# zhengxwen/HIBAG

Measured on AMD Instinct MI355X. Metric: hlaPredict() samples/sec, 10k samples x 100-classifier HLA-B, higher is better.
Workload: dtype f64; 1 GPU; BASELINE config 2: synthetic hla-b model (50 alleles, 100 classifiers, 150 SNPs, 505000 haplotype-pair evaluations/sample), 10000 samples per GPU per step, type=response+dosage, vote=prob; genotypes and outputs resident in HBM (transfers excluded: `host_inclusive` is the PCIe-inclusive rate of the host-pointer entry); samples_per_gpu=10000, parallelism=sample-sharded x1 (contiguous slices, no collective), kernel_target=HIP, gfx950:sramecc+:xnack-, AMD Radeon Graphics, 256 CUs, engine=mfma (FP4 / int8 MFMA distances + FP64 VALU accumulation in reference order)

## Files before the change

### hibag_amd/_lib.py

```python

from __future__ import annotations

import ctypes as C
import os
import subprocess

_HERE = os.path.dirname(os.path.abspath(__file__))
CSRC = os.path.join(_HERE, "csrc")
LIB_PATH = os.environ.get("HIBAG_HIP_LIBRARY") or os.path.join(CSRC, "libhibag_hip.so")

K_PACK, K_TOTAL, K_ACCUM, K_FINISH, K_COUNT = 0, 1, 2, 3, 4
KERNEL_NAMES = {K_PACK: "pack", K_TOTAL: "total", K_ACCUM: "accum", K_FINISH: "finish"}

EXPORTS = [
    "hibag_hip_abi_version", "hibag_hip_last_error", "hibag_hip_device_count", "hibag_hip_set_device", "hibag_hip_get_device",
    "hibag_hip_set_kernel_target", "hibag_hip_model_new", "hibag_hip_model_add_classifier",
    "hibag_hip_model_add_classifier_packed", "hibag_hip_model_finalize", "hibag_hip_model_free",
    "hibag_hip_model_n_hla", "hibag_hip_model_n_snp", "hibag_hip_model_n_classifier",
    "hibag_hip_model_pair_evals", "hibag_hip_model_stored_cells", "hibag_hip_model_second_pass_pairs", "hibag_hip_model_mutation_table", "hibag_hip_predict",
    "hibag_hip_predict_device", "hibag_hip_model_set_snp_weights", "hibag_hip_predict_partial_device",
    "hibag_hip_finish_device", "hibag_hip_set_timing", "hibag_hip_get_timing", "hibag_hip_reset_timing",
    "hibag_hip_gpu_ext_proc", "hibag_hip_bed_flag", "hibag_hip_conv_bed", "hibag_hip_predict_bed", "hibag_hip_predict_mapped", "hibag_hip_predict_mapped_device",
    "hibag_hip_predict_snp_major", "hibag_hip_predict_snp_major_device",
    "hibag_hip_trainer_new", "hibag_hip_trainer_free", "hibag_hip_trainer_set_rng", "hibag_hip_trainer_set_seed",
    "hibag_hip_trainer_new_classifiers", "hibag_hip_trainer_n_classifier", "hibag_hip_trainer_classifier_dims",
    "hibag_hip_trainer_classifier_get", "hibag_hip_trainer_set_threads", "hibag_hip_trainer_threads", "hibag_hip_trainer_set_em_mode",
    "hibag_hip_trainer_set_shared", "hibag_hip_train_set_thread_budget", "hibag_hip_train_combine_stats", "hibag_hip_train_combine_times",
    "hibag_hip_model_status", "hibag_hip_model_clear_status", "hibag_hip_model_handover_faults",
    "hibag_hip_test_inject_handover_fault", "hibag_hip_model_engine", "hibag_hip_model_replicate",
    "hibag_hip_multi_slice", "hibag_hip_predict_multi", "hibag_hip_model_device",
    "hibag_hip_shard_bounds", "hibag_hip_model_shard", "hibag_hip_model_batch_limit", "hibag_hip_shard_group_new",
    "hibag_hip_shard_group_free", "hibag_hip_shard_group_ranks", "hibag_hip_shard_group_allreduces", "hibag_hip_rccl_version",
    "hibag_hip_shard_group_predict", "hibag_hip_predict_multi_sharded", "hibag_hip_measure_issue_costs",
    "hibag_hip_test_time_avg_prob", "hibag_hip_test_read_diag", "hibag_hip_plugin_degraded_calls", "hibag_hip_predict_oob",
    "hibag_hip_ld_geno_new", "hibag_hip_ld_geno_free", "hibag_hip_ld_snp_counts", "hibag_hip_ld_matrix", "hibag_hip_ld_gram_ms",
    "hibag_hip_ld_hla", "hibag_hip_model_distance", "hibag_hip_model_distance_ms",
    "hibag_hip_merge_plan_new", "hibag_hip_merge_plan_free", "hibag_hip_merge_device", "hibag_hip_predict_merge",
    "hibag_hip_predict_merge_bed", "hibag_hip_predict_prefix", "hibag_hip_predict_prefix_ms",
    "hibag_hip_predict_topk", "hibag_hip_predict_topk_device", "hibag_hip_predict_topk_mapped",
    "hibag_hip_predict_topk_snp_major", "hibag_hip_predict_topk_bed",
    "hibag_hip_cohort_new", "hibag_hip_cohort_from_bed", "hibag_hip_cohort_free", "hibag_hip_cohort_device",
    "hibag_hip_cohort_n_samp", "hibag_hip_cohort_n_snp", "hibag_hip_cohort_bytes", "hibag_hip_cohort_snp_counts",
    "hibag_hip_predict_cohort", "hibag_hip_predict_topk_cohort", "hibag_hip_predict_masked",
    "hibag_hip_test_build_eval_batch",
]
TOPK_MAX = 16


class HibagHipError(RuntimeError):
    def __init__(self, code: int, message: str):
        super().__init__(message or f"libhibag_hip error {code}")
        self.code = code


def build(force: bool = False) -> str:
    cmd = ["make", "-C", CSRC, "-s", "-j2"] + (["-B"] if force else [])
    subprocess.check_call(cmd)
    return LIB_PATH


_lib = None


def lib() -> C.CDLL:
    global _lib
    if _lib is not None:
        return _lib
# ... 110 lines not shown
    L.hibag_hip_model_engine.argtypes = [vp, i32, C.POINTER(i32), C.POINTER(i32)]
    L.hibag_hip_model_replicate.argtypes = [vp, i32]
    L.hibag_hip_model_replicate.restype = vp
    L.hibag_hip_multi_slice.argtypes = [i32, i32, i32, C.POINTER(i32), C.POINTER(i32)]
    L.hibag_hip_predict_multi.argtypes = [C.POINTER(vp), i32, vp, i32, i32, vp, vp, vp, vp, vp, vp]
    L.hibag_hip_shard_bounds.argtypes = [i32, i32, i32, C.POINTER(i32), C.POINTER(i32)]
    L.hibag_hip_model_shard.argtypes = [vp, i32, i32, i32]
    L.hibag_hip_model_shard.restype = vp
    L.hibag_hip_model_batch_limit.argtypes = [vp]
    L.hibag_hip_shard_group_new.argtypes = [C.POINTER(vp), i32]
    L.hibag_hip_shard_group_new.restype = vp
    L.hibag_hip_shard_group_free.argtypes = [vp]
    L.hibag_hip_shard_group_free.restype = None
    L.hibag_hip_shard_group_ranks.argtypes = [vp]
    L.hibag_hip_shard_group_allreduces.argtypes = [vp]
    L.hibag_hip_shard_group_allreduces.restype = i64
    L.hibag_hip_rccl_version.restype = i32
    L.hibag_hip_shard_group_predict.argtypes = [vp, vp, i32, vp, vp, vp, vp, vp, vp]
    L.hibag_hip_predict_multi_sharded.argtypes = [C.POINTER(vp), i32, vp, i32, vp, vp, vp, vp, vp, vp]
    L.hibag_hip_measure_issue_costs.argtypes = [C.POINTER(dbl)] * 4
    L.hibag_hip_test_time_avg_prob.argtypes = [vp, vp, i32, i32, i32, vp, vp, C.POINTER(dbl)]
    if hasattr(L, "hibag_hip_test_build_eval_batch"):
        L.hibag_hip_test_build_eval_batch.argtypes = [i32, i32, vp, vp, i32, i32, vp, vp, vp, vp, i32, vp, i32, vp, vp]
    if hasattr(L, "hibag_hip_test_read_diag"):
        L.hibag_hip_test_read_diag.argtypes = [vp, vp, i32]
        L.hibag_hip_plugin_degraded_calls.restype = i64
    _lib = L
    return L


def check(rc: int) -> None:
    if rc != 0:
        raise HibagHipError(rc, lib().hibag_hip_last_error().decode("utf-8", "replace"))
```

### hibag_amd/csrc/hibag_internal.h

```cpp
#ifndef HIBAG_INTERNAL_H_
#define HIBAG_INTERNAL_H_

#include <hip/hip_runtime.h>
#include <algorithm>
#include <chrono>
#include <cmath>
#include <cstdarg>
#include <cstdio>
#include <cstdlib>
#include <cstring>
#include <mutex>
#include <new>
#include <string>
#include <thread>
#include <vector>

#include "../../include/hibag_hip.h"
#include "hibag_device.h"
#include "hibag_kernels.h"
#include "hibag_plugin.h"

int hibag_fail(int code, const char *fmt, ...);
int hibag_selected_device();

// ... 122 lines not shown

}
using namespace hibag_detail;

struct hibag_hip_model {
	int device = 0;
	int n_hla = 0, n_snp = 0;
	bool finalized = false;
	bool have_snpidx = true;
	bool use_mfma = true;
	bool use_fp4 = true;
	std::vector<HostClassifier> cls;
	std::vector<int> snp_weight_override;
	int64_t pair_evals = 0;
	double tab[HIBAG_TAB_N];

	DevBuf d_int, d_stream, d_tile, d_tab, d_blk, d_pfac, d_phdr, d_parow;
	HibagModelView view{};
	int mask_rows = 0, bt_rows = 0, cell_rows = 0;
	size_t stream_bytes = 0;

	DevBuf ws_planes, ws_cw, ws_tot, ws_inv, ws_winv, ws_part, ws_best, ws_vrec, ws_geno, ws_out, ws_codes, ws_bt, ws_bias, ws_cells, ws_sync;
	std::vector<int> engine_of, steps_of;
	int store_mode = 0;
	int64_t second_pass_pairs = 0;
	HibagSideStream side;
	uint32_t epoch = 0;
	int *h_err = nullptr;
	DevBuf ws_err;
	int fault = 0;
	int64_t fault_count = 0;
	bool no_chunks = false;
	int drop_next = 0;
	uint32_t spin_limit = 1u << 19;
	hipEvent_t ws_done = nullptr;
	bool ws_pending = false;
	StagedStreams staged;
	PinBuf pin_geno, pin_out;
	bool staged_ready = false;
	DevBuf ws_bed, ws_bedidx;
	DevBuf oob_hap;
	size_t oob_freq_at = 0, oob_off_at = 0, oob_start_at = 0;
	bool oob_hap_ready = false;
	hipStream_t dist_st = nullptr;
	hipEvent_t dist_ev[2] = {nullptr, nullptr};
	DevBuf dist_cells, dist_tri, dist_acc, dist_num, dist_out;
// ... 84 lines not shown
```

### hibag_amd/csrc/hibag_k_pass1.h

```cpp
#ifndef HIBAG_K_PASS1_H_
#define HIBAG_K_PASS1_H_

__device__ __forceinline__ double *cell_rows(const HibagModelView &M, const HibagBatchView &B, int c, int group)
{
	return B.cells + ((size_t)group * (size_t)M.cell_row[M.n_classifier] + (size_t)M.cell_row[c]) * HIBAG_WAVE;
}

template <int NWP>
__device__ __forceinline__ double classifier_total(const HibagModelView &M, const HibagBatchView &B,
	int c, int s, int i0, int i1, int chunk0, double *__restrict__ rows, const double *tab_s)
{
	LaneMask<NWP> L;
	load_masks<NWP>(B, M.mask_row[c], s, L);
	const uint32_t *__restrict__ cnt = M.cls_cnt + M.cls_off[c];
	const uint32_t *__restrict__ cp = M.stream + M.stream_off[c] + (size_t)chunk0 * HIBAG_CHUNK_DWORDS(NWP);
	double total = 0;
	uint32_t n = cnt[i0];
	for (int i = i0; i < i1; i++) {
		const uint32_t n_next = cnt[i + 1];
		const double cell = cell_sum<NWP>(n, cp, L, tab_s);
		if (rows) __builtin_nontemporal_store(cell, &rows[(size_t)i * HIBAG_WAVE + (s & 63)]);
		total += cell;
		n = n_next;
	}
// ... 177 lines not shown
	double cell = 0, total = 0;
	double *__restrict__ rows = cell_rows(M, B, c, group);
	int row = seg[1];
	auto fin = [&](double v, bool, int) {
		__builtin_nontemporal_store(v, &rows[(size_t)row * HIBAG_WAVE + lane]); row++;
		if (WHOLE) { total += v; asm("" : "+v"(total)); }
	};
	const WideSrc wide = wide_src(B, M.bt_row[c], M.n_step[c], group);
	LaneOperand T;
	load_operand_row<HIBAG_ENGINE_FP4W>(B, M.bt_row[c], c, group, lane, T);
	ListCursor cur;
	walk_blocks<HIBAG_ENGINE_FP4W, TOTAL_G, false>(M, M.wide_seg_off[blockIdx.y], seg[2], lane, cur, hap_rsrc(M, M.hap_off[c]),
		M.n_snp_c[c] - HIBAG_FP4_STEP_SNPS * (wide.nstep - 1), T, wide, tab_s, cell, fin);
	if (WHOLE) {
		const size_t at = (size_t)c * B.n_pad + s;
		const double inv = 1 / total;
		B.tot[at] = total;
		B.inv[at] = inv;
		B.winv[2 * at + 1] = B.cw[at] > 0 ? inv : 0.0;
		note_infinite_reciprocal(B, c, s, B.cw[at], inv);
	}
}

__global__ void k_total_scan(HibagModelView M, HibagBatchView B)
{
	const int c = M.split_cls[blockIdx.y];
	const int s = blockIdx.x * blockDim.x + threadIdx.x;
	if (s >= B.n_pad) return;
	const double *__restrict__ rows = cell_rows(M, B, c, s >> 6) + (s & 63);
	const int n = M.cls_n[c];
	double total = 0;
	int i = 0;
	for (; i + 32 <= n; i += 32) {
		double v[32];
#pragma unroll
		for (int j = 0; j < 32; j++) v[j] = rows[(size_t)(i + j) * HIBAG_WAVE];
#pragma unroll
		for (int j = 0; j < 32; j++) total += v[j];
	}
	for (; i < n; i++) total += rows[(size_t)i * HIBAG_WAVE];
	B.tot[(size_t)c * B.n_pad + s] = total;
	B.inv[(size_t)c * B.n_pad + s] = 1 / total;
	B.winv[2 * ((size_t)c * B.n_pad + s) + 1] = B.cw[(size_t)c * B.n_pad + s] > 0 ? 1 / total : 0.0;
	note_infinite_reciprocal(B, c, s, B.cw[(size_t)c * B.n_pad + s], 1 / total);
}

template <int NB = 16>
__device__ __forceinline__ void ensemble_scalars(const HibagModelView &M, const HibagBatchView &B, int s, const int *__restrict__ best_cell)
{
	double sum_w = 0, sum_m = 0, num_m = 0;
	for (int c0 = 0; c0 < M.n_classifier; c0 += NB) {
		double wv[NB], tv[NB];
		int bv[NB];
#pragma unroll
		for (int j = 0; j < NB; j++) {
			const bool in = c0 + j < M.n_classifier;
			const size_t at = (size_t)(in ? c0 + j : c0) * B.n_pad + s;
			wv[j] = in ? B.cw[at] : 0.0;
			tv[j] = B.tot[at];
			bv[j] = best_cell ? best_cell[at] : 0;
		}
#pragma unroll
		for (int j = 0; j < NB; j++) {
// ... 23 lines not shown
```

### hibag_amd/csrc/hibag_kernels.hip

```cpp

#include <hip/hip_runtime.h>
#include <stdint.h>
#include <stdlib.h>
#include <string.h>
#include <algorithm>
#include "hibag_device.h"
#include "hibag_kernels.h"

#define NA_INTEGER (-2147483647 - 1)
#define CH HIBAG_CHUNK
#define BLOCK_WAVES HIBAG_BLOCK_WAVES
#define BLOCK_THREADS (BLOCK_WAVES * HIBAG_WAVE)
#ifndef TOTAL_G
#define TOTAL_G 8
#endif
#ifndef HIBAG_TOT_OCC
#define HIBAG_TOT_OCC 5
#endif
#ifndef HIBAG_TOT_OCC_MANY
#define HIBAG_TOT_OCC_MANY 6
#endif
#ifndef ACCUM_AHEAD
#define ACCUM_AHEAD true
#endif
// ... 94 lines not shown
{
	total[0] = resident_blocks(k_total<false, HIBAG_TOT_OCC, 0>, BLOCK_THREADS);
	total[1] = resident_blocks(k_total<false, HIBAG_TOT_OCC_MANY, 2>, BLOCK_THREADS);
	total[2] = resident_blocks(k_total<true, HIBAG_TOT_OCC, 0>, BLOCK_THREADS);
	total[3] = resident_blocks(k_total<true, HIBAG_TOT_OCC_MANY, 2>, BLOCK_THREADS);
	*accum = resident_blocks(k_accum, ACCUM_WAVES * HIBAG_WAVE);
}

void hibag_launch_total(const HibagModelView &M, const HibagBatchView &B, hipStream_t st, const HibagSideStream &side, bool vote)
{
	if (M.n_classifier == 0) return;
	const bool wide = M.n_wide > 0;
	if (wide) {
		const unsigned gq = (unsigned)((B.n_pad / HIBAG_WAVE + BLOCK_WAVES - 1) / BLOCK_WAVES);
		HibagModelView W = M;
		W.split_cls = M.wide_scan;
		const hipStream_t ws = side.stream ? side.stream : st;
		if (side.stream) {
			(void)hipEventRecord(side.fork, st);
			(void)hipStreamWaitEvent(side.stream, side.fork, 0);
		}
		if (M.n_wide_seg > 0 && M.n_wide_scan < M.n_wide) hipLaunchKernelGGL(k_total_wide<true>, dim3(gq, M.n_wide_seg), dim3(BLOCK_THREADS), 0, ws, M, B);
		else if (M.n_wide_seg > 0) hipLaunchKernelGGL(k_total_wide<false>, dim3(gq, M.n_wide_seg), dim3(BLOCK_THREADS), 0, ws, M, B);
		if (M.n_wide_scan > 0) hipLaunchKernelGGL(k_total_scan, dim3(B.n_pad / 64, M.n_wide_scan), dim3(64), 0, ws, W, B);
		if (side.stream) (void)hipEventRecord(side.join, side.stream);
	}
	if (M.n_item_whole == 0) {
		if (wide && side.stream) (void)hipStreamWaitEvent(st, side.join, 0);
		return;
	}
	const unsigned gx = (unsigned)((B.n_pad / HIBAG_WAVE + BLOCK_WAVES - 1) / BLOCK_WAVES);
	HibagModelView V = M;
	const double groups = (double)(B.n_pad / HIBAG_WAVE);
	const bool split = M.n_split > 0 && 1.25 * M.split_heavy_ns > M.split_rest_ns * groups / 4096.0;
	V.item = split ? M.item_split : M.item_whole;
	V.n_item = split ? M.n_item_split : M.n_item_whole;
	if (!split) V.n_split = 0;
	const unsigned n = gx * (unsigned)V.n_item;
	const int sbase = (M.store_cells && !vote) ? 2 : 0;
	const int slots_many = M.slots_total[sbase + 1];
	const bool many = M.all_fp4 && !split && slots_many > 0 && n >= 2u * (unsigned)slots_many;
	const int slots = M.slots_total[sbase + (many ? 1 : 0)];
	unsigned n_whole = n, rest = 0, stride = 8, K = 1;
	const int k_pass1 = tail_chunks(B.tail_k, M.p1_blocks / std::max(M.n_classifier, 1));
	if (!vote && k_pass1 > 1 && slots > 0 && n > (unsigned)slots) {
		K = (unsigned)k_pass1;
		rest = n % (unsigned)slots + (unsigned)slots;
		n_whole = n - rest;
		stride = (rest + 7) / 8 * 8;
	}
	const dim3 grid(n_whole + (rest ? K * stride : 0));
#define LAUNCH_TOTAL(STORE, OCC, WALK, VOTE) hipLaunchKernelGGL((k_total<STORE, OCC, WALK, VOTE>), grid, dim3(BLOCK_THREADS), 0, st, V, B, (int)gx, (int)n_whole, (int)rest, (int)stride, (int)K)
#define LAUNCH_WALK(STORE, VOTE) do { if (!many) LAUNCH_TOTAL(STORE, HIBAG_TOT_OCC, 0, VOTE);                                 \
		else if (M.p1_prebuilt) LAUNCH_TOTAL(STORE, HIBAG_TOT_OCC_MANY, 2, VOTE); else LAUNCH_TOTAL(STORE, HIBAG_TOT_OCC_MANY, 1, VOTE); } while (0)
	if (vote) LAUNCH_WALK(false, true);
	else if (M.store_cells) LAUNCH_WALK(true, false);
	else LAUNCH_WALK(false, false);
#undef LAUNCH_WALK
#undef LAUNCH_TOTAL
	if (split)
		hipLaunchKernelGGL(k_total_scan, dim3(B.n_pad / 64, V.n_split), dim3(64), 0, st, V, B);
	if (wide && side.stream) (void)hipStreamWaitEvent(st, side.join, 0);
}

void hibag_launch_accum(const HibagModelView &M, const HibagBatchView &B, hipStream_t st)
{
	if (M.store_cells == 1 && M.n_classifier > 0) {
		const unsigned groups_x = (unsigned)((B.n_pad / HIBAG_WAVE + 7) / 8), tq = (unsigned)((M.n_tile + CELLS_WAVES - 1) / CELLS_WAVES);
		hipLaunchKernelGGL(k_accum_cells, dim3(8 * groups_x * tq), dim3(CELLS_WAVES * HIBAG_WAVE), 0, st, M, B);
		return;
	}
	const unsigned n_group = (unsigned)(B.n_pad / HIBAG_WAVE);
	const unsigned n = 8u * (((n_group + 7) / 8 + ACCUM_WAVES - 1) / ACCUM_WAVES) * (unsigned)M.n_tile;
	if (n == 0 || M.n_classifier == 0) {
		(void)hipMemsetAsync(B.part, 0, (size_t)M.n_cell * B.n_pad * sizeof(double), st);
		return;
	}
	const int slots = M.slots_accum;
	const unsigned nx = n / 8, sx = (unsigned)slots / 8;
	unsigned n_whole = nx, K = 1;
	if (tail_chunks(B.tail_k, 0, 2) > 1 && sx > 0 && nx > sx) {
		K = (unsigned)tail_chunks(B.tail_k, 0, 2);
		n_whole = nx - (nx % sx + sx);
	}
// ... 77 lines not shown
```

### hibag_amd/csrc/hibag_model.hip

```cpp

#include "hibag_internal.h"

namespace hibag_detail {

void build_table(double *tab)
{
	const double min_rare_freq = 1e-5;
	for (int i = 0; i < HIBAG_TAB_N; i++) tab[i] = std::exp(i * std::log(min_rare_freq));
	tab[0] = 1;
	for (int i = 0; i < HIBAG_TAB_N; i++)
		if (!std::isfinite(tab[i])) tab[i] = 0;
}

int check_classifier_args(hibag_hip_model *m, int n_snp_c, const int32_t *snpidx, int n_haplo,
	const double *freq, const int32_t *hla)
{
	if (!m) return hibag_fail(HIBAG_HIP_EINVAL, "model is NULL");
	if (m->finalized) return hibag_fail(HIBAG_HIP_ESTATE, "model already finalized");
	if (n_snp_c < 0 || n_snp_c > HIBAG_HIP_MAX_SNP_IN_CLASSIFIER)
		return hibag_fail(HIBAG_HIP_EINVAL, "there are too many SNP markers in a classifier (%d > %d).",
			n_snp_c, HIBAG_HIP_MAX_SNP_IN_CLASSIFIER);
	if (n_haplo < 0 || (n_haplo > 0 && (!freq || !hla)))
		return hibag_fail(HIBAG_HIP_EINVAL, "invalid haplotype list");
	if (snpidx)
		for (int i = 0; i < n_snp_c; i++)
			if (snpidx[i] < 0 || snpidx[i] >= m->n_snp)
// ... 171 lines not shown
struct ModelLayout {
	struct ClassifierPlan {
		std::vector<int> st;
		std::vector<uint32_t> chunks, npairs;
		std::vector<uint8_t> stored;
		int64_t pairs = 0;
	};
	struct SlotRange { size_t first, n; int c; };
	int C, nh, S, P;
	std::vector<ClassifierPlan> cp;
	std::vector<int> n_snp_c, nwp, snp_off, mask_row, c_order, snp_index, snp_weight, engine, bt_row, cls_nblk, n_step;
	std::vector<uint64_t> stream_off, cell_work;
	std::vector<uint32_t> stream, hap, hap_off;
	int rows = 0, bt_rows = 0;
	int64_t pair_evals = 0;
	std::vector<int> tile_p0, tile_n, tile_h1, tile_h2;
	int n_tile = 0, store_mode = 0;
	std::vector<uint32_t> cls_cnt, cls_cell, tile_meta, tile_k0, tile_nlist, tile_nstored;
	std::vector<uint64_t> tile_jpack;
	std::vector<int> cls_off, cls_n, n_stored_c;
	int64_t second_pass_pairs = 0;
	std::vector<int> item, item_whole, split_row, split_cls, wide_cls;
	double split_heavy_ns = 0, split_rest_ns = 0;
	std::vector<uint32_t> plist, ehdr, etile_cstart, blk_close;
	std::vector<uint64_t> etile_blk0, blk_off, wseg_off;
	std::vector<SlotRange> slot_ranges;
	std::vector<int> cell_row, wseg, wide_scan;
	uint64_t estream_blocks = 0, p1_base = 0;
	long long p1_blocks = 0;
	std::vector<double> pfac;
	std::vector<uint32_t> phdr, parow, ctile;
	size_t parow_blocks = 0;
	bool p1_prebuilt = false;
	explicit ModelLayout(const hibag_hip_model *m)
		: C((int)m->cls.size()), nh(m->n_hla), S(m->n_snp), P(nh * (nh + 1) / 2), cp(C), n_snp_c(C), nwp(C), snp_off(C), mask_row(C),
		  c_order(C), snp_weight(std::max(S, 1), 0), engine(std::max(C, 1), 0), bt_row(std::max(C, 1), 0), cls_nblk(std::max(C, 1), 0),
		  n_step(std::max(C, 1), 1), stream_off(std::max(C, 1), 0), cell_work(P, 0), hap_off(std::max(C, 1), 0) {}
	bool evaluates(int c) const { return engine[c] == HIBAG_ENGINE_FP4 && n_step[c] == 1; }
	bool stored_big(int c, int p) const { return store_mode == 2 && cp[c].stored[p] != 0; }
};

void append_hap_entry(const HostClassifier &k, int engine, int steps, double ff, int i, double f, std::vector<uint32_t> &hap)
{
	const bool fp4 = engine == HIBAG_ENGINE_FP4;
	auto window = [&](int i, int lo) -> uint32_t {
		if (i < 0) return 0u;
// ... 193 lines not shown
			L.tile_nlist[ct] = (uint32_t)nl;
			L.tile_nstored[ct] = (uint32_t)ns;
			L.tile_k0[ct] = (uint32_t)(L.store_mode == 2 ? L.n_stored_c[c] : k_first);
			L.n_stored_c[c] += ns;
			k_first += k;
			for (int j = 0; j < L.tile_n[t]; j++)
				if (!chunks[p0 + j]) me[4 + k++] = (uint32_t)j << 24;
		}
	}
	if (L.cls_cnt.empty()) { L.cls_cnt.push_back(0); L.cls_cell.push_back(0); }
	return 0;
}

void plan_work_items(ModelLayout &L)
{
	L.split_row.assign(std::max(L.C, 1), -1);
	std::vector<double> work(L.C, 0.0);
	double typical = 0;
	int n_typ = 0;
	for (int c = 0; c < L.C; c++) {
		work[c] = (double)L.cp[c].pairs * (L.engine[c] ? 50.0 * (0.5 + 0.5 * L.n_step[c]) : 48.0 * L.nwp[c]);
		if (L.engine[c]) { typical += work[c]; n_typ++; }
		L.split_rest_ns += work[c];
	}
	typical = n_typ ? typical / n_typ : 0;
	std::vector<std::pair<double, std::vector<int>>> items, whole;
	for (int c = 0; c < L.C; c++) {
		if (L.n_step[c] > 1) { L.wide_cls.push_back(c); continue; }
		const int n = L.cls_n[c];
		const uint32_t *cnt = &L.cls_cnt[L.cls_off[c]];
		whole.push_back({work[c], {c, 0, n, 0}});
		int nseg = 1;
		if (!L.engine[c] && typical > 0 && work[c] > 3 * typical)
			nseg = (int)std::min<double>(64, std::max(2.0, std::floor(work[c] / typical)));
		if (nseg == 1 || n < 2) {
			items.push_back({work[c], {c, 0, n, 0}});
			continue;
		}
		L.split_heavy_ns = std::max(L.split_heavy_ns, (double)L.cp[c].pairs * 18.0 * L.nwp[c]);
		L.split_row[c] = 1;
		L.split_cls.push_back(c);
		uint64_t total = 0, acc = 0, chunk0 = 0;
		for (int i = 0; i < n; i++) total += cnt[i] + 1;
		int i0 = 0, k = 1;
		for (int i = 0; i < n; i++) {
			acc += cnt[i] + 1;
// ... 49 lines not shown
							jp >>= 4;
						}
				const int nsb = std::max(0, std::min(HIBAG_STORED_PER_VISIT, ns - HIBAG_STORED_PER_VISIT * b));
				if (c > 0xFFFF) return hibag_fail(HIBAG_HIP_EINVAL, "too many classifiers (%d) for the second pass's block headers", C);
				const uint32_t bt = (uint32_t)(HIBAG_ENGINE_ROWS(L.engine[c], L.n_snp_c[c]) > 0 ? L.bt_row[c] : 0);
				if (bt > 0xFFFFu) return hibag_fail(HIBAG_HIP_EINVAL, "too many classifiers for the matrix engine's operand rows");
				const uint32_t h[8] = {
					(uint32_t)c | (bt << 16), srow | ((uint32_t)nsb << 25),
					0u, 0u,
					(uint32_t)jq, (uint32_t)(jq >> 32),
					(uint32_t)jps, 0u};
				ehdr.insert(ehdr.end(), h, h + 8);
				jps >>= 4 * nsb;
				srow += (uint32_t)nsb;
			}
		}
		L.etile_cstart[(size_t)t * (C + 1) + C] = (uint32_t)(plist.size() / HIBAG_PLIST_DWORDS - L.etile_blk0[t]);
	}
	L.estream_blocks = plist.size() / HIBAG_PLIST_DWORDS + 4;
	plist.insert(plist.end(), 4 * HIBAG_PLIST_DWORDS, 0u);
	ehdr.resize(L.estream_blocks * 8, 0u);
	L.p1_base = plist.size();
	L.blk_off.assign(std::max(C, 1), 0);
	for (int c = 0; c < C; c++) {
		if (!L.engine[c]) continue;
		const uint32_t pad = (uint32_t)m->cls[c].freq.size();
		L.blk_off[c] = plist.size();
		if (L.n_step[c] > 1) {
			const bool whole = (int)L.wide_cls.size() >= 8;
			const long long seg_pairs = whole ? (1ll << 62) : std::max<long long>(512, 6000 / L.n_step[c]);
			bool any_seg = false;
			int p_lo = 0, h1_lo = 0, h2_lo = 0, row = 0, h1 = 0, h2 = 0;
			long long acc_pairs = 0;
			int rows_in_seg = 0;
			for (int p = 0; p < L.P; p++) {
				acc_pairs += L.cp[c].npairs[p];
				rows_in_seg += L.cp[c].npairs[p] != 0;
				int nh1 = h1, nh2 = h2 + 1;
				if (nh2 == L.nh) { nh1++; nh2 = nh1; }
				if (acc_pairs >= seg_pairs || p + 1 == L.P) {
					const size_t off = plist.size();
					const int nb = append_pair_blocks(L.cp[c].st.data(), L.nh, h1_lo, h2_lo, p_lo, p + 1 - p_lo, pad, plist, L.cp[c].stored.data(), nullptr);
					if (nb > 0) { L.wseg.insert(L.wseg.end(), {c, row, nb, whole ? 1 : 0}); L.wseg_off.push_back(off); any_seg = true; }
					row += rows_in_seg; rows_in_seg = 0; acc_pairs = 0;
					p_lo = p + 1; h1_lo = nh1; h2_lo = nh2;
				}
				h1 = nh1; h2 = nh2;
			}
			if (!whole || !any_seg) L.wide_scan.push_back(c);
		} else
			append_pair_blocks(L.cp[c].st.data(), L.nh, 0, 0, 0, L.P, pad, plist, L.store_mode ? L.cp[c].stored.data() : nullptr, nullptr);
		L.cls_nblk[c] = (int)((plist.size() - L.blk_off[c]) / HIBAG_PLIST_DWORDS);
		L.slot_ranges.push_back({(size_t)L.blk_off[c], plist.size() - (size_t)L.blk_off[c], c});
		L.p1_blocks += L.cls_nblk[c];
		uint32_t closed = 0;
		for (int b = 0; b < L.cls_nblk[c] && L.store_mode; b++) {
			L.blk_close.push_back(L.n_step[c] > 1 ? 0u : closed);
			for (int i = 0; i < HIBAG_PLIST_DWORDS; i++) closed += (plist[L.blk_off[c] + (size_t)b * HIBAG_PLIST_DWORDS + i] >> 30) & 1u;
		}
	}
	if (L.blk_close.empty()) L.blk_close.push_back(0);
	plist.insert(plist.end(), 4 * HIBAG_PLIST_DWORDS, 0u);
	return 0;
}

void plan_factors(const hibag_hip_model *m, ModelLayout &L)
{
	L.pfac.assign(L.plist.size(), 0.0);
	for (const auto &r : L.slot_ranges) {
		const std::vector<double> &freq = m->cls[r.c].freq;
		const uint32_t H = (uint32_t)freq.size();
		auto ff_of = [&](uint32_t e) { return e < H ? 2 * freq[e] : e == H ? 0.0 : freq[e - H - 1]; };
// ... 134 lines not shown
	}
	V.split_heavy_ns = L.split_heavy_ns; V.split_rest_ns = L.split_rest_ns;
	V.hap_dwords = (uint32_t)L.hap.size();
	V.estream_blocks = L.estream_blocks;
	V.p1_base = L.p1_base;
	V.p1_blocks = L.p1_blocks;
	V.store_cells = L.store_mode;
	hibag_query_slots(V.slots_total, &V.slots_accum);
	V.plist_dwords = L.plist.size();
	V.parow_blocks = L.parow_blocks;
	V.p1_prebuilt = L.p1_prebuilt ? 1 : 0;
	long long longest = 0;
	for (int c = 0; c < L.C; c++) longest = std::max<long long>(longest, L.engine[c] ? L.cls_nblk[c] : L.cp[c].pairs / 8);
	m->spin_limit = (uint32_t)std::min<long long>(0xFFFFFFF0ll, (1ll << 19) + 16 * longest);
	m->pair_evals = L.pair_evals;
	m->store_mode = L.store_mode;
	m->second_pass_pairs = L.second_pass_pairs;
	m->cell_rows = L.cell_row[L.C];
	m->bt_rows = L.bt_rows;
	m->mask_rows = L.rows;
	m->stream_bytes = L.stream.size() * sizeof(uint32_t);
	m->engine_of.assign(L.engine.begin(), L.engine.begin() + L.C);
	m->steps_of.assign(L.n_step.begin(), L.n_step.begin() + L.C);
	m->finalized = true;
	return 0;
}

static int finalize_with(hibag_hip_model *m, const FinalizeOptions &opt)
{
	if (m->finalized) return hibag_fail(HIBAG_HIP_ESTATE, "model already finalized");
	ModelLayout L(m);
	if (int rc = plan_classifiers(m, opt, L)) return rc;
	plan_tiles(L);
	plan_store(opt, L);
	if (int rc = plan_cell_lists(L)) return rc;
	plan_work_items(L);
	if (int rc = plan_pair_lists(m, L)) return rc;
	plan_factors(m, L);
	plan_parow(opt, L);
	if (int rc = plan_ctile(L)) return rc;
	return upload_layout(m, L);
}

int finalize_model(hibag_hip_model *m) { return finalize_with(m, FinalizeOptions()); }

int finalize_model_stream(hibag_hip_model *m)
// ... 153 lines not shown
		m->have_snpidx = src->have_snpidx; m->use_mfma = src->use_mfma; m->use_fp4 = src->use_fp4;
		m->cls.assign(src->cls.begin() + first, src->cls.begin() + first + count);
		if (!src->snp_weight_override.empty()) m->snp_weight_override = src->snp_weight_override;
		else {
			m->snp_weight_override.assign(std::max(src->n_snp, 1), 0);
			for (const HostClassifier &k : src->cls)
				for (int v : k.snpidx) m->snp_weight_override[v]++;
		}
		memcpy(m->tab, src->tab, sizeof(m->tab));
	} catch (...) { delete m; hibag_fail(HIBAG_HIP_ENOMEM, "out of host memory"); return nullptr; }
	if (src->finalized && hibag_hip_model_finalize(m)) { delete m; return nullptr; }
	return m;
}

int hibag_hip_model_engine(const hibag_hip_model *m, int classifier, int *engine, int *k_steps)
{
	if (!m || !m->finalized) return hibag_fail(HIBAG_HIP_ESTATE, "model not finalized");
	if (classifier < 0 || classifier >= (int)m->cls.size()) return hibag_fail(HIBAG_HIP_EINVAL, "classifier %d out of range", classifier);
	if (engine) *engine = m->engine_of[classifier];
	if (k_steps) *k_steps = m->steps_of[classifier];
	return 0;
}

}
```

### hibag_amd/hibag.py

```python

from __future__ import annotations

import ctypes as C
import os
import sys
from typing import List, Optional, Sequence, Union

import numpy as np

from . import _lib
from ._lib import HibagHipError
from .bed import HlaBEDGeno
from .cohort import HlaDeviceCohort
from .model import (NA_INTEGER, Classifier, HlaAttrBagObj, HlaSNPGeno)

_TARGETS_CPU = ("max", "auto.avx2", "base", "sse2", "sse4", "avx", "avx2", "avx512f", "avx512bw",
                "avx512vpopcnt")
_kernel_target: Optional[str] = None
_kernel_info: str = ""


def hlaSetKernelTarget(cpu: str = "hip") -> List[str]:
    global _kernel_target, _kernel_info
    cpu = str(cpu)
# ... 85 lines not shown

    def stored_cells(self) -> int:
        return int(_lib.lib().hibag_hip_model_stored_cells(self.handle))

    def second_pass_pairs(self) -> int:
        return int(_lib.lib().hibag_hip_model_second_pass_pairs(self.handle))

    def status(self) -> int:
        return int(_lib.lib().hibag_hip_model_status(self.handle))

    def clear_status(self):
        _lib.check(_lib.lib().hibag_hip_model_clear_status(self.handle))

    def handover_faults(self) -> int:
        return int(_lib.lib().hibag_hip_model_handover_faults(self.handle))

    def inject_handover_fault(self, which_pass: int):
        _lib.check(_lib.lib().hibag_hip_test_inject_handover_fault(self.handle, int(which_pass)))

    def engine(self, classifier: int):
        e, k = C.c_int(0), C.c_int(0)
        _lib.check(_lib.lib().hibag_hip_model_engine(self.handle, int(classifier), C.byref(e), C.byref(k)))
        return {0: "valu", 1: "fp4", 2: "i8", 3: "i8"}[e.value], k.value

    def replicate(self, device: int) -> "HlaAttrBagClass":
        h = _lib.lib().hibag_hip_model_replicate(self.handle, int(device))
        if not h:
            raise HibagHipError(-2, _lib.lib().hibag_hip_last_error().decode())
        r = object.__new__(HlaAttrBagClass)
        r.obj = self.obj
        r._h = C.c_void_p(h)
        return r

    def shard(self, shard: int, n_shards: int, device: int) -> "HlaAttrBagClass":
        h = _lib.lib().hibag_hip_model_shard(self.handle, int(shard), int(n_shards), int(device))
        if not h:
            raise HibagHipError(-2, _lib.lib().hibag_hip_last_error().decode())
        r = object.__new__(HlaAttrBagClass)
        r.obj = self.obj
        r._h = C.c_void_p(h)
        return r

    def mutation_table(self) -> np.ndarray:
        t = np.empty(257, np.float64)
        _lib.check(_lib.lib().hibag_hip_model_mutation_table(self.handle, _as_ptr(t)))
        return t
# ... 627 lines not shown
```

### include/hibag_hip.h

```cpp
#ifndef HIBAG_HIP_H_
#define HIBAG_HIP_H_

#include <stddef.h>
#include <stdint.h>

#ifdef __cplusplus
extern "C" {
#endif

#define HIBAG_HIP_ABI_VERSION 7

#define HIBAG_HIP_OK          0
#define HIBAG_HIP_EINVAL     (-1)
#define HIBAG_HIP_ENODEV     (-2)
#define HIBAG_HIP_ENOMEM     (-3)
#define HIBAG_HIP_ESTATE     (-4)
#define HIBAG_HIP_EHANDOVER  (-5)

#define HIBAG_HIP_NA_INTEGER (-2147483647 - 1)

#define HIBAG_HIP_MAX_SNP_IN_CLASSIFIER 128

typedef struct hibag_hip_model hibag_hip_model;

// ... 86 lines not shown
	double *d_matching, double *d_dosage, double *d_postprob, void *stream);

int hibag_hip_predict_mapped(hibag_hip_model *m, const int32_t *geno, int n_samp, int n_geno_snp,
	const int32_t *snp_col, const int32_t *flip, int vote_method,
	int32_t *H1, int32_t *H2, double *max_prob, double *matching, double *dosage, double *postprob);
int hibag_hip_predict_mapped_device(hibag_hip_model *m, const int32_t *d_geno, int n_samp, int n_geno_snp,
	const int32_t *d_snp_col, const int32_t *d_flip, int vote_method,
	int32_t *d_H1, int32_t *d_H2, double *d_max_prob, double *d_matching, double *d_dosage,
	double *d_postprob, void *stream);

int hibag_hip_predict_snp_major(hibag_hip_model *m, const int32_t *geno, size_t ld, int n_samp, int n_geno_snp,
	const int32_t *snp_col, const int32_t *flip, int vote_method,
	int32_t *H1, int32_t *H2, double *max_prob, double *matching, double *dosage, double *postprob);
int hibag_hip_predict_snp_major_device(hibag_hip_model *m, const int32_t *d_geno, size_t ld, int n_samp, int n_geno_snp,
	const int32_t *d_snp_col, const int32_t *d_flip, int vote_method,
	int32_t *d_H1, int32_t *d_H2, double *d_max_prob, double *d_matching, double *d_dosage,
	double *d_postprob, void *stream);

int hibag_hip_model_status(hibag_hip_model *m);
int hibag_hip_model_clear_status(hibag_hip_model *m);
int64_t hibag_hip_model_handover_faults(const hibag_hip_model *m);
int hibag_hip_test_inject_handover_fault(hibag_hip_model *m, int pass);
int hibag_hip_test_read_diag(hibag_hip_model *m, unsigned long long *out, int n);

#define HIBAG_HIP_ENGINE_VALU 0
#define HIBAG_HIP_ENGINE_FP4  1
#define HIBAG_HIP_ENGINE_I8   2
#define HIBAG_HIP_ENGINE_I8S  3
int hibag_hip_model_engine(const hibag_hip_model *m, int classifier, int *engine, int *k_steps);

hibag_hip_model *hibag_hip_model_replicate(const hibag_hip_model *m, int device);
int hibag_hip_multi_slice(int n_samp, int n_models, int i, int *first, int *count);
int hibag_hip_predict_multi(hibag_hip_model *const *models, int n_models, const int32_t *geno, int n_samp,
	int vote_method, int32_t *H1, int32_t *H2, double *max_prob, double *matching, double *dosage, double *postprob);

int hibag_hip_model_set_snp_weights(hibag_hip_model *m, const int32_t *snp_weight);
int hibag_hip_predict_partial_device(hibag_hip_model *m, const int32_t *d_geno,
	int n_samp, double *d_partial, void *stream);
int hibag_hip_finish_device(hibag_hip_model *m, const double *d_partial, int n_samp,
	int32_t *d_H1, int32_t *d_H2, double *d_max_prob, double *d_matching,
	double *d_dosage, double *d_postprob, void *stream);

typedef struct hibag_hip_shard_group hibag_hip_shard_group;
int hibag_hip_shard_bounds(int n_classifier, int n_shards, int shard, int *first, int *count);
hibag_hip_model *hibag_hip_model_shard(const hibag_hip_model *src, int shard, int n_shards, int device);
int hibag_hip_model_batch_limit(const hibag_hip_model *m);
// ... 108 lines not shown
```

Baseline: 8.115 million samples/s.

## Spread wide-classifier total scan over four waves and size wide segments by blocks

The total-scan kernel now launches four waves per block. Each wave loads a slice of 64 cell rows into LDS, and wave 0 sums them in order, so memory loads are issued in parallel while the FP64 summation order stays the same. Segmentation of wide (multi-step) classifiers moves into a helper header that targets a block count per segment. It picks a longer segment form when narrow work greatly outweighs wide work, letting fewer, larger segments hide behind the narrow pass. The change adds LDS use, a per-tile barrier and test hooks for forcing the form, and risks idle waves during the serial sum.

```diff
diff --git a/hibag_amd/_lib.py b/hibag_amd/_lib.py
--- a/hibag_amd/_lib.py
+++ b/hibag_amd/_lib.py
@@ -42,7 +42,7 @@
     "hibag_hip_cohort_new", "hibag_hip_cohort_from_bed", "hibag_hip_cohort_free", "hibag_hip_cohort_device",
     "hibag_hip_cohort_n_samp", "hibag_hip_cohort_n_snp", "hibag_hip_cohort_bytes", "hibag_hip_cohort_snp_counts",
     "hibag_hip_predict_cohort", "hibag_hip_predict_topk_cohort", "hibag_hip_predict_masked",
-    "hibag_hip_test_build_eval_batch",
+    "hibag_hip_test_build_eval_batch", "hibag_hip_test_set_wide_form", "hibag_hip_test_wide_segments",
 ]
 TOPK_MAX = 16
 
@@ -199,6 +199,9 @@
     L.hibag_hip_test_time_avg_prob.argtypes = [vp, vp, i32, i32, i32, vp, vp, C.POINTER(dbl)]
     if hasattr(L, "hibag_hip_test_build_eval_batch"):
         L.hibag_hip_test_build_eval_batch.argtypes = [i32, i32, vp, vp, i32, i32, vp, vp, vp, vp, i32, vp, i32, vp, vp]
+    if hasattr(L, "hibag_hip_test_set_wide_form"):
+        L.hibag_hip_test_set_wide_form.argtypes = [i32]
+        L.hibag_hip_test_wide_segments.argtypes = [vp, vp, i32]
     if hasattr(L, "hibag_hip_test_read_diag"):
         L.hibag_hip_test_read_diag.argtypes = [vp, vp, i32]
         L.hibag_hip_plugin_degraded_calls.restype = i64
diff --git a/hibag_amd/csrc/hibag_internal.h b/hibag_amd/csrc/hibag_internal.h
--- a/hibag_amd/csrc/hibag_internal.h
+++ b/hibag_amd/csrc/hibag_internal.h
@@ -168,6 +168,7 @@
 
 	DevBuf ws_planes, ws_cw, ws_tot, ws_inv, ws_winv, ws_part, ws_best, ws_vrec, ws_geno, ws_out, ws_codes, ws_bt, ws_bias, ws_cells, ws_sync;
 	std::vector<int> engine_of, steps_of;
+	std::vector<int> wide_seg_of;
 	int store_mode = 0;
 	int64_t second_pass_pairs = 0;
 	HibagSideStream side;
diff --git a/hibag_amd/csrc/hibag_k_pass1.h b/hibag_amd/csrc/hibag_k_pass1.h
--- a/hibag_amd/csrc/hibag_k_pass1.h
+++ b/hibag_amd/csrc/hibag_k_pass1.h
@@ -223,23 +223,46 @@
 	}
 }
 
-__global__ void k_total_scan(HibagModelView M, HibagBatchView B)
-{
+#ifndef SCAN_WAVES
+#define SCAN_WAVES 4
+#define SCAN_ROWS 64
+#endif
+#define SCAN_PER_WAVE (SCAN_ROWS / SCAN_WAVES)
+__global__ __launch_bounds__(SCAN_WAVES * HIBAG_WAVE) void k_total_scan(HibagModelView M, HibagBatchView B)
+{
+	__shared__ double turn_s[SCAN_ROWS][HIBAG_WAVE];
 	const int c = M.split_cls[blockIdx.y];
-	const int s = blockIdx.x * blockDim.x + threadIdx.x;
-	if (s >= B.n_pad) return;
-	const double *__restrict__ rows = cell_rows(M, B, c, s >> 6) + (s & 63);
+	const int wave = __builtin_amdgcn_readfirstlane(threadIdx.x >> 6), lane = threadIdx.x & 63;
+	const int s = blockIdx.x * HIBAG_WAVE + lane;
+	if (blockIdx.x * HIBAG_WAVE >= B.n_pad) return;
+	const double *__restrict__ rows = cell_rows(M, B, c, blockIdx.x) + lane;
 	const int n = M.cls_n[c];
-	double total = 0;
-	int i = 0;
-	for (; i + 32 <= n; i += 32) {
-		double v[32];
-#pragma unroll
-		for (int j = 0; j < 32; j++) v[j] = rows[(size_t)(i + j) * HIBAG_WAVE];
-#pragma unroll
-		for (int j = 0; j < 32; j++) total += v[j];
-	}
-	for (; i < n; i++) total += rows[(size_t)i * HIBAG_WAVE];
+	double total = 0, v[SCAN_PER_WAVE];
+	auto request = [&](int i) {
+#pragma unroll
+		for (int j = 0; j < SCAN_PER_WAVE; j++) {
+			const int r = i + wave * SCAN_PER_WAVE + j;
+			v[j] = r < n ? rows[(size_t)r * HIBAG_WAVE] : 0.0;
+		}
+	};
+	request(0);
+	for (int i = 0; i < n; i += SCAN_ROWS) {
+#pragma unroll
+		for (int j = 0; j < SCAN_PER_WAVE; j++) turn_s[wave * SCAN_PER_WAVE + j][lane] = v[j];
+		__syncthreads();
+		if (i + SCAN_ROWS < n) request(i + SCAN_ROWS);
+		if (wave == 0) {
+			const int m = min(SCAN_ROWS, n - i);
+			int j = 0;
+			for (; j + 16 <= m; j += 16) {
+#pragma unroll
+				for (int k = 0; k < 16; k++) total += turn_s[j + k][lane];
+			}
+			for (; j < m; j++) total += turn_s[j][lane];
+		}
+		__syncthreads();
+	}
+	if (wave != 0) return;
 	B.tot[(size_t)c * B.n_pad + s] = total;
 	B.inv[(size_t)c * B.n_pad + s] = 1 / total;
 	B.winv[2 * ((size_t)c * B.n_pad + s) + 1] = B.cw[(size_t)c * B.n_pad + s] > 0 ? 1 / total : 0.0;
diff --git a/hibag_amd/csrc/hibag_kernels.hip b/hibag_amd/csrc/hibag_kernels.hip
--- a/hibag_amd/csrc/hibag_kernels.hip
+++ b/hibag_amd/csrc/hibag_kernels.hip
@@ -140,7 +140,7 @@
 		}
 		if (M.n_wide_seg > 0 && M.n_wide_scan < M.n_wide) hipLaunchKernelGGL(k_total_wide<true>, dim3(gq, M.n_wide_seg), dim3(BLOCK_THREADS), 0, ws, M, B);
 		else if (M.n_wide_seg > 0) hipLaunchKernelGGL(k_total_wide<false>, dim3(gq, M.n_wide_seg), dim3(BLOCK_THREADS), 0, ws, M, B);
-		if (M.n_wide_scan > 0) hipLaunchKernelGGL(k_total_scan, dim3(B.n_pad / 64, M.n_wide_scan), dim3(64), 0, ws, W, B);
+		if (M.n_wide_scan > 0) hipLaunchKernelGGL(k_total_scan, dim3(B.n_pad / 64, M.n_wide_scan), dim3(SCAN_WAVES * HIBAG_WAVE), 0, ws, W, B);
 		if (side.stream) (void)hipEventRecord(side.join, side.stream);
 	}
 	if (M.n_item_whole == 0) {
@@ -177,7 +177,7 @@
 #undef LAUNCH_WALK
 #undef LAUNCH_TOTAL
 	if (split)
-		hipLaunchKernelGGL(k_total_scan, dim3(B.n_pad / 64, V.n_split), dim3(64), 0, st, V, B);
+		hipLaunchKernelGGL(k_total_scan, dim3(B.n_pad / 64, V.n_split), dim3(SCAN_WAVES * HIBAG_WAVE), 0, st, V, B);
 	if (wide && side.stream) (void)hipStreamWaitEvent(st, side.join, 0);
 }
 
diff --git a/hibag_amd/csrc/hibag_model.hip b/hibag_amd/csrc/hibag_model.hip
--- a/hibag_amd/csrc/hibag_model.hip
+++ b/hibag_amd/csrc/hibag_model.hip
@@ -1,7 +1,14 @@
 
 #include "hibag_internal.h"
+#include "hibag_wide_seg.h"
+#include <atomic>
+
+static_assert(HIBAG_PLIST_DWORDS == HIBAG_WIDE_SLOTS_PER_BLOCK, "hibag_wide_seg.h counts blocks of HIBAG_PLIST_DWORDS slots");
 
 namespace hibag_detail {
+
+static std::atomic<int> g_wide_form{-1};
+void set_wide_form(int form) { g_wide_form.store(form < 0 || form > HIBAG_WIDE_FORM_LONG ? -1 : form); }
 
 void build_table(double *tab)
 {
@@ -219,6 +226,7 @@
 	int64_t second_pass_pairs = 0;
 	std::vector<int> item, item_whole, split_row, split_cls, wide_cls;
 	double split_heavy_ns = 0, split_rest_ns = 0;
+	double narrow_ns = 0, wide_ns = 0;
 	std::vector<uint32_t> plist, ehdr, etile_cstart, blk_close;
 	std::vector<uint64_t> etile_blk0, blk_off, wseg_off;
 	std::vector<SlotRange> slot_ranges;
@@ -458,6 +466,7 @@
 		work[c] = (double)L.cp[c].pairs * (L.engine[c] ? 50.0 * (0.5 + 0.5 * L.n_step[c]) : 48.0 * L.nwp[c]);
 		if (L.engine[c]) { typical += work[c]; n_typ++; }
 		L.split_rest_ns += work[c];
+		(L.n_step[c] > 1 ? L.wide_ns : L.narrow_ns) += work[c];
 	}
 	typical = n_typ ? typical / n_typ : 0;
 	std::vector<std::pair<double, std::vector<int>>> items, whole;
@@ -553,32 +562,30 @@
 	ehdr.resize(L.estream_blocks * 8, 0u);
 	L.p1_base = plist.size();
 	L.blk_off.assign(std::max(C, 1), 0);
+	std::vector<std::pair<int, int>> cell_h;
 	for (int c = 0; c < C; c++) {
 		if (!L.engine[c]) continue;
 		const uint32_t pad = (uint32_t)m->cls[c].freq.size();
 		L.blk_off[c] = plist.size();
 		if (L.n_step[c] > 1) {
-			const bool whole = (int)L.wide_cls.size() >= 8;
-			const long long seg_pairs = whole ? (1ll << 62) : std::max<long long>(512, 6000 / L.n_step[c]);
-			bool any_seg = false;
-			int p_lo = 0, h1_lo = 0, h2_lo = 0, row = 0, h1 = 0, h2 = 0;
-			long long acc_pairs = 0;
-			int rows_in_seg = 0;
-			for (int p = 0; p < L.P; p++) {
-				acc_pairs += L.cp[c].npairs[p];
-				rows_in_seg += L.cp[c].npairs[p] != 0;
-				int nh1 = h1, nh2 = h2 + 1;
-				if (nh2 == L.nh) { nh1++; nh2 = nh1; }
-				if (acc_pairs >= seg_pairs || p + 1 == L.P) {
-					const size_t off = plist.size();
-					const int nb = append_pair_blocks(L.cp[c].st.data(), L.nh, h1_lo, h2_lo, p_lo, p + 1 - p_lo, pad, plist, L.cp[c].stored.data(), nullptr);
-					if (nb > 0) { L.wseg.insert(L.wseg.end(), {c, row, nb, whole ? 1 : 0}); L.wseg_off.push_back(off); any_seg = true; }
-					row += rows_in_seg; rows_in_seg = 0; acc_pairs = 0;
-					p_lo = p + 1; h1_lo = nh1; h2_lo = nh2;
-				}
-				h1 = nh1; h2 = nh2;
+			const int form = hibag_wide_form((int)L.wide_cls.size(), L.narrow_ns, L.wide_ns, g_wide_form.load());
+			const bool whole = form == HIBAG_WIDE_FORM_WHOLE;
+			if (cell_h.empty()) {
+				cell_h.reserve((size_t)L.P);
+				for (int a = 0; a < L.nh; a++)
+					for (int b = a; b < L.nh; b++) cell_h.push_back({a, b});
 			}
-			if (!whole || !any_seg) L.wide_scan.push_back(c);
+			const std::vector<HibagWideSegment> segs = hibag_wide_segments(L.cp[c].npairs.data(), L.P, hibag_wide_target_blocks(form, L.n_step[c]));
+			for (const HibagWideSegment &s : segs) {
+				const size_t off = plist.size();
+				const int nb = append_pair_blocks(L.cp[c].st.data(), L.nh, cell_h[s.cell0].first, cell_h[s.cell0].second, s.cell0, s.n_cells, pad,
+					plist, L.cp[c].stored.data(), nullptr);
+				if (nb != (int)((s.slots + HIBAG_PLIST_DWORDS - 1) / HIBAG_PLIST_DWORDS))
+					return hibag_fail(HIBAG_HIP_ESTATE, "internal: a segment of classifier %d has %d blocks for %lld slots", c, nb, s.slots);
+				L.wseg.insert(L.wseg.end(), {c, s.row0, nb, whole ? 1 : 0});
+				L.wseg_off.push_back(off);
+			}
+			if (!whole || segs.empty()) L.wide_scan.push_back(c);
 		} else
 			append_pair_blocks(L.cp[c].st.data(), L.nh, 0, 0, 0, L.P, pad, plist, L.store_mode ? L.cp[c].stored.data() : nullptr, nullptr);
 		L.cls_nblk[c] = (int)((plist.size() - L.blk_off[c]) / HIBAG_PLIST_DWORDS);
@@ -759,6 +766,7 @@
 	m->stream_bytes = L.stream.size() * sizeof(uint32_t);
 	m->engine_of.assign(L.engine.begin(), L.engine.begin() + L.C);
 	m->steps_of.assign(L.n_step.begin(), L.n_step.begin() + L.C);
+	m->wide_seg_of = L.wseg;
 	m->finalized = true;
 	return 0;
 }
@@ -958,4 +966,18 @@
 	return 0;
 }
 
-}
+int hibag_hip_test_set_wide_form(int form)
+{
+	set_wide_form(form);
+	return 0;
+}
+
+int hibag_hip_test_wide_segments(const hibag_hip_model *m, int32_t *out, int cap)
+{
+	if (!m || !m->finalized) return hibag_fail(HIBAG_HIP_ESTATE, "model not finalized");
+	const int n = (int)(m->wide_seg_of.size() / 4);
+	for (int i = 0; out && i < std::min(n, cap) * 4; i++) out[i] = m->wide_seg_of[i];
+	return n;
+}
+
+}
diff --git a/hibag_amd/csrc/hibag_wide_seg.h b/hibag_amd/csrc/hibag_wide_seg.h
--- /dev/null
+++ b/hibag_amd/csrc/hibag_wide_seg.h
@@ -0,0 +1,51 @@
+#ifndef HIBAG_WIDE_SEG_H_
+#define HIBAG_WIDE_SEG_H_
+
+#include <cstdint>
+#include <vector>
+
+#ifndef HIBAG_WIDE_SEG_BLOCKS
+#define HIBAG_WIDE_SEG_BLOCKS 8
+#endif
+inline int hibag_wide_seg_blocks_hidden(int k_steps) { return k_steps > 0 && 188 / k_steps > 16 ? 188 / k_steps : 16; }
+#define HIBAG_WIDE_HIDDEN_RATIO 32
+inline bool hibag_wide_hidden(double narrow_work, double wide_work) { return narrow_work >= HIBAG_WIDE_HIDDEN_RATIO * wide_work; }
+#define HIBAG_WIDE_WHOLE_MIN 8
+#define HIBAG_WIDE_SLOTS_PER_BLOCK 32
+enum { HIBAG_WIDE_FORM_SHORT = 0, HIBAG_WIDE_FORM_WHOLE = 1, HIBAG_WIDE_FORM_LONG = 2 };
+
+struct HibagWideSegment { int cell0, n_cells, row0; long long slots; };
+
+inline int hibag_wide_form(int n_wide_classifiers, double narrow_work, double wide_work, int forced = -1)
+{
+	if (forced >= 0) return forced;
+	if (n_wide_classifiers >= HIBAG_WIDE_WHOLE_MIN) return HIBAG_WIDE_FORM_WHOLE;
+	return hibag_wide_hidden(narrow_work, wide_work) ? HIBAG_WIDE_FORM_LONG : HIBAG_WIDE_FORM_SHORT;
+}
+inline int hibag_wide_target_blocks(int form, int k_steps)
+{
+	return form == HIBAG_WIDE_FORM_WHOLE ? 0 : form == HIBAG_WIDE_FORM_LONG ? hibag_wide_seg_blocks_hidden(k_steps) : HIBAG_WIDE_SEG_BLOCKS;
+}
+
+inline std::vector<HibagWideSegment> hibag_wide_segments(const uint32_t *npairs, int n_cells, int target_blocks)
+{
+	std::vector<HibagWideSegment> segs;
+	const long long target = target_blocks > 0 ? (long long)target_blocks * HIBAG_WIDE_SLOTS_PER_BLOCK : (1ll << 62);
+	HibagWideSegment s = {0, 0, 0, 0};
+	int rows = 0;
+	for (int p = 0; p < n_cells; p++) {
+		s.n_cells++;
+		s.slots += (long long)npairs[p] + (npairs[p] & 1u);
+		rows += npairs[p] != 0;
+		if (s.slots >= target || p + 1 == n_cells) {
+			if (s.slots > 0) segs.push_back(s);
+			else if (!segs.empty()) segs.back().n_cells += s.n_cells;
+			else continue;
+			s = HibagWideSegment{p + 1, 0, s.row0 + rows, 0};
+			rows = 0;
+		}
+	}
+	return segs;
+}
+
+#endif
diff --git a/hibag_amd/hibag.py b/hibag_amd/hibag.py
--- a/hibag_amd/hibag.py
+++ b/hibag_amd/hibag.py
@@ -131,6 +131,16 @@
         e, k = C.c_int(0), C.c_int(0)
         _lib.check(_lib.lib().hibag_hip_model_engine(self.handle, int(classifier), C.byref(e), C.byref(k)))
         return {0: "valu", 1: "fp4", 2: "i8", 3: "i8"}[e.value], k.value
+
+    def wide_segments(self):
+        L = _lib.lib()
+        n = L.hibag_hip_test_wide_segments(self.handle, None, 0)
+        if n < 0:
+            _lib.check(n)
+        out = np.zeros((n, 4), dtype=np.int32)
+        if n:
+            L.hibag_hip_test_wide_segments(self.handle, out.ctypes.data_as(C.c_void_p), n)
+        return out
 
     def replicate(self, device: int) -> "HlaAttrBagClass":
         h = _lib.lib().hibag_hip_model_replicate(self.handle, int(device))
diff --git a/include/hibag_hip.h b/include/hibag_hip.h
--- a/include/hibag_hip.h
+++ b/include/hibag_hip.h
@@ -132,6 +132,8 @@
 int64_t hibag_hip_model_handover_faults(const hibag_hip_model *m);
 int hibag_hip_test_inject_handover_fault(hibag_hip_model *m, int pass);
 int hibag_hip_test_read_diag(hibag_hip_model *m, unsigned long long *out, int n);
+int hibag_hip_test_set_wide_form(int form);
+int hibag_hip_test_wide_segments(const hibag_hip_model *m, int32_t *out, int cap);
 
 #define HIBAG_HIP_ENGINE_VALU 0
 #define HIBAG_HIP_ENGINE_FP4  1
```

Result: no change. 8.064 million samples/s (-0.6%).
